# simongroeger/irm_motion_planning

Hardware: AMD Instinct MI355X
Metric: GD iterations/sec (batch of trajectories) (higher is better)
Workload: dtype f32

## Files before the change

### irm_motion_planning_amd/csrc/irm_kernels_impl.hpp

```cpp
#pragma once
#include <hip/hip_runtime.h>
#include <math.h>
#include <stdint.h>
#include <stdio.h>

#include <type_traits>

#include "irm_kernels.hpp"

namespace irm {

typedef float f32x4 __attribute__((ext_vector_type(4)));
typedef float f32x2 __attribute__((ext_vector_type(2)));

__device__ __forceinline__ f32x2 pkfma(f32x2 a, f32x2 b, f32x2 c) { return __builtin_elementwise_fma(a, b, c); }


template <int CTRL>
__device__ __forceinline__ float dppf(float v) {
    static_assert(CTRL == 0xB1 || CTRL == 0x4E || CTRL == 0x141 || CTRL == 0x140, "in-row permutations only");
    return __int_as_float(__builtin_amdgcn_mov_dpp(__float_as_int(v), CTRL, 0xF, 0xF, true));
}
template <int CTRL>
__device__ __forceinline__ int dppi(int v) {
// ... 2626 lines not shown
                } else {
                    G = *reinterpret_cast<const f32x4*>(Gb + ycl * lde + u * 16 + r4y);
                }
                tile(u, G, fresh, *reinterpret_cast<const f32x4*>(Ab + ycl * lde + u * 16 + r4y),
                     vt_frag(u));
            }
        }
        *reinterpret_cast<f32x4*>(Zq + pz * 256 + (r4 >> 2) * 64 + cl * 4) = acc0 + acc1;
    };
    auto bls_f = [&]() {
        const float* zq = Zq + (r4 >> 2) * 64 + cl * 4;
        f32x4 by0, bz;
        if constexpr (kBFix) {
            f32x4 yp[S::NSPLIT], zz[kNZc];
#pragma unroll
            for (int sp = 0; sp < S::NSPLIT; ++sp) yp[sp] = *reinterpret_cast<const f32x4*>(Ypart + (sp * 16 + ycl) * ldy + r4y);
#pragma unroll
            for (int w = 0; w < kNZc; ++w) zz[w] = *reinterpret_cast<const f32x4*>(zq + w * 256);
            __builtin_amdgcn_sched_barrier(0);
            by0 = yp[0];
#pragma unroll
            for (int sp = 1; sp < S::NSPLIT; ++sp) by0 += yp[sp];
            bz = zz[0];
#pragma unroll
            for (int w = 1; w < kNZc; ++w) bz += zz[w];
        } else {
            by0 = *reinterpret_cast<const f32x4*>(Ypart + ycl * ldy + r4y);
            for (int sp = 1; sp < nsplit; ++sp) by0 += *reinterpret_cast<const f32x4*>(Ypart + (sp * 16 + ycl) * ldy + r4y);
            bz = *reinterpret_cast<const f32x4*>(zq);
            for (int w = 1; w < nzp; ++w) bz += *reinterpret_cast<const f32x4*>(zq + w * 256);
        }
        const f32x4 bt = by0 + bz;
        f32x4 acc[S2T];
#pragma unroll
        for (int j = 0; j < S2T; ++j) {
            acc[j] = f32x4{0.f, 0.f, 0.f, 0.f};
            if (wave + j * nwaves < MT2) {
#pragma unroll
                for (int m = 0; m < 4; ++m) acc[j] = __builtin_amdgcn_mfma_f32_16x16x4f32(a2[j * 2][m], bt[m], acc[j], 0, 0, 0);
            }
        }
#pragma unroll
        for (int j = 0; j < S2T; ++j)
            if (wave + j * nwaves < MT2) *reinterpret_cast<f32x4*>(dP + cl * ldx + (wave + j * nwaves) * 16 + r4x) = acc[j];
    };
    constexpr int kDW = MAXT / 64;
    constexpr int kD1 = DENSE ? (S::RP / 16 + kDW - 1) / kDW : 1;
    constexpr int kD2 = DENSE ? (S::MP / 16 + kDW - 1) / kDW : 1;
    constexpr int kDQ = DENSE ? S::NK / 16 : 1;
    constexpr int kDPF = 2;
    float aepd[kD1];
#pragma unroll
    for (int j = 0; j < kD1; ++j) {
        const int tl = wave + j * kDW;
        aepd[j] = 0.f;
        if (DENSE && tl < RP / 16 && (lane >> 4) < 2) aepd[j] = P.Fbot[(size_t)((lane >> 4) ? N - 1 : 0) * RP + tl * 16 + (lane & 15)];
    }
    auto dense_stage1 = [&](bool full) {
        const f32x4 z4 = {0.f, 0.f, 0.f, 0.f};
        constexpr int KQ1c = S::MP / 16;
        const __amdgpu_buffer_rsrc_t r1 = __builtin_amdgcn_make_buffer_rsrc(
            const_cast<float*>(P.F1p), 0, (int)(frag_floats(S::RP, S::MP) * 4), 0x00020000);
        const int vo = lane * 16;
        auto g1ld = [&](int tl, int kq) { return ld_frag(r1, vo, ((tl * KQ1c + kq) * 64) * 16); };
        const float* xl = X + cl * ldx + r4x;
        const float bep = smem[epoff];
        f32x4 acc[kD1];
#pragma unroll
        for (int j = 0; j < kD1; ++j) acc[j] = __builtin_amdgcn_mfma_f32_16x16x4f32(aepd[j], bep, z4, 0, 0, 0);
        auto half = [&](int kb) {
            f32x4 a[kDPF][kD1], b[kDPF];
#pragma unroll
            for (int p = 0; p < kDPF; ++p) {
#pragma unroll
                for (int j = 0; j < kD1; ++j) a[p][j] = g1ld(wave + j * kDW, kb + p);
                b[p] = *reinterpret_cast<const f32x4*>(xl + (kb + p) * 16);
            }
#pragma unroll
            for (int kq = 0; kq < kDQ; ++kq) {
                const int sl = kq % kDPF;
                f32x4 ac[kD1];
#pragma unroll
                for (int j = 0; j < kD1; ++j) ac[j] = a[sl][j];
                const f32x4 bc = b[sl];
                if (kq + kDPF < kDQ) {
#pragma unroll
                    for (int j = 0; j < kD1; ++j) a[sl][j] = g1ld(wave + j * kDW, kb + kq + kDPF);
                    b[sl] = *reinterpret_cast<const f32x4*>(xl + (kb + kq + kDPF) * 16);
                }
#pragma unroll
                for (int m = 0; m < 4; ++m)
#pragma unroll
                    for (int j = 0; j < kD1; ++j) acc[j] = __builtin_amdgcn_mfma_f32_16x16x4f32(ac[j][m], bc[m], acc[j], 0, 0, 0);
                __builtin_amdgcn_sched_barrier(0);
            }
        };
        half(0);
        if (full) half(kDQ);
#pragma unroll
        for (int j = 0; j < kD1; ++j)
            *reinterpret_cast<f32x4*>(Ypart + cl * ldy + (wave + j * kDW) * 16 + r4x) = acc[j];
    };
    auto dense_stage2 = [&]() {
        constexpr int KQ2c = S::RP / 16;
        const __amdgpu_buffer_rsrc_t r2 = __builtin_amdgcn_make_buffer_rsrc(
            const_cast<float*>(P.F2p), 0, (int)(frag_floats(S::MP, S::RP) * 4), 0x00020000);
        const int vo = lane * 16;
        auto g2ld = [&](int tl, int kq) { return ld_frag(r2, vo, ((tl * KQ2c + kq) * 64) * 16); };
        const float* yl = Ypart + cl * ldy + r4x;
        const float* el = Eb + cl * lde + r4x;
        f32x4 acc[kD2], a[kDPF][kD2], by[kDPF], be[kDPF];
#pragma unroll
        for (int j = 0; j < kD2; ++j) acc[j] = f32x4{0.f, 0.f, 0.f, 0.f};
#pragma unroll
        for (int p = 0; p < kDPF; ++p) {
#pragma unroll
            for (int j = 0; j < kD2; ++j) a[p][j] = g2ld(wave + j * kDW, p);
            by[p] = *reinterpret_cast<const f32x4*>(yl + p * 16);
            be[p] = *reinterpret_cast<const f32x4*>(el + p * 16);
        }
#pragma unroll
        for (int kq = 0; kq < kDQ; ++kq) {
            const int sl = kq % kDPF;
            f32x4 ac[kD2];
#pragma unroll
            for (int j = 0; j < kD2; ++j) ac[j] = a[sl][j];
            const f32x4 bt = by[sl] + be[sl];
            if (kq + kDPF < kDQ) {
#pragma unroll
                for (int j = 0; j < kD2; ++j) a[sl][j] = g2ld(wave + j * kDW, kq + kDPF);
                by[sl] = *reinterpret_cast<const f32x4*>(yl + (kq + kDPF) * 16);
                be[sl] = *reinterpret_cast<const f32x4*>(el + (kq + kDPF) * 16);
            }
#pragma unroll
            for (int m = 0; m < 4; ++m)
#pragma unroll
                for (int j = 0; j < kD2; ++j) acc[j] = __builtin_amdgcn_mfma_f32_16x16x4f32(ac[j][m], bt[m], acc[j], 0, 0, 0);
            __builtin_amdgcn_sched_barrier(0);
        }
#pragma unroll
        for (int j = 0; j < kD2; ++j)
            *reinterpret_cast<f32x4*>(dP + cl * ldx + (wave + j * kDW) * 16 + r4x) = acc[j];
    };
    auto direction = [&](int j, float (&dt)[D], float (&dv)[D]) {
        float ut[D], uv[D];
#pragma unroll
        for (int k = 0; k < D; ++k) {
            ut[k] = dP[(t * D + k) * ldx + swz(nn[j], t * D + k)];
            uv[k] = dP[(t * D + k) * ldx + NK + swz(nn[j], t * D + k)];
        }
#pragma unroll
        for (int k = 0; k < D; ++k) {
            float a = ut[0] * P.J[k], c = uv[0] * P.J[k];
#pragma unroll
            for (int l = 1; l < D; ++l) {
                a = fmaf(ut[l], P.J[l * D + k], a);
                c = fmaf(uv[l], P.J[l * D + k], c);
            }
            dt[k] = a;
            dv[k] = c;
        }
    };
    auto grad_alpha = [&](int j, float (&G)[D], int gt) {
        const int r = wl[j] ? nn[j] : 0;
#pragma unroll
        for (int k = 0; k < D; ++k) {
            if constexpr (DENSE) G[k] = Ypart[(gt * D + k) * ldy + swz(r, gt * D + k)];
            else G[k] = Gb[(gt * D + k) * lde + swz(r, gt * D + k)];
        }
    };
    auto ser_row = [&](int j) {
        int r = nn[j] * D;
        if constexpr (D > 3) asm volatile("" : "+v"(r));
        return r;
    };
    auto snapshot = [&](irm_stats& st) {
        if (rec && st.series_len < P.max_series) {
#pragma unroll
            for (int j = 0; j < WPL; ++j) {
                if (vl[j]) {
#pragma unroll
                    for (int k = 0; k < D; ++k)
                        P.series[((b * P.max_series) + st.series_len) * N * D + ser_row(j) + k] = q[j][k];
                }
            }
            st.series_len++;
        }
    };

    float* SS = smem + LX.ss;
    float* HP = smem + LX.hp;
    constexpr int kSlots = (MAXT / 64) / WPTL;
    auto ss_write = [&](int tt, const float (&a)[WPL][D], const float (&qq)[WPL][D], const float (&vv)[WPL][D]) {
        const int th = tt * NWL + li;
#pragma unroll
        for (int k = 0; k < D; ++k) {
            SS[k * MAXT + th] = a[0][k];
            SS[(D + k) * MAXT + th] = qq[0][k];
            SS[(2 * D + k) * MAXT + th] = vv[0][k];
        }
    };
    auto ss_read = [&](int tt) {
        const int th = tt * NWL + li;
#pragma unroll
        for (int k = 0; k < D; ++k) {
            al[0][k] = SS[k * MAXT + th];
            q[0][k] = SS[(D + k) * MAXT + th];
            v[0][k] = SS[(2 * D + k) * MAXT + th];
        }
    };
    bool adopt = false;
    bool qpend = false;
    auto ts_write = [&]() {
        if (n0 == 0 && lane == 0) {
            TS[t * kTsW + 0] = lr;
            TS[t * kTsW + 2] = phase == LP_STEP ? 1.f : 0.f;
            if constexpr (QUE) TS[t * kTsW + 3] = __int_as_float((int)b);
        }
    };
    int n_rounds = 0, n_hm = 0;

    irm_stats st{};
    st.series_len = rec ? 1 : 0;
    if constexpr (BLS && D <= 3) {
        asm volatile("" : "+v"(st.inner_iterations), "+v"(st.outer_iterations), "+v"(st.grad_evals), "+v"(st.cost_evals),
                     "+v"(st.bls_trials), "+v"(st.series_len), "+v"(n_rounds), "+v"(n_hm));
    }
    auto write_out = [&]() {
#pragma unroll
        for (int j = 0; j < WPL; ++j) {
            if (vl[j]) {
#pragma unroll
                for (int k = 0; k < D; ++k) {
                    if (P.traj_out) P.traj_out[(b * N + nn[j]) * D + k] = q[j][k];
                    if (P.alpha_out) P.alpha_out[(b * N + nn[j]) * D + k] = al[j][k];
                }
            }
        }
        if (P.stats && li == 0) P.stats[b] = st;
    };

    float loss;
    bool done = !tvalid;
    {
        WP<D> w[WPL];
        evaluate(q, v, false, ljl, w);
        __syncthreads();
        const Fin f = finalize(lsg, t);
        loss = f.nl;
        if constexpr (!BLS) st.cost_evals = 1;
        bool to_end = P.max_inner <= 0;
        if constexpr (BLS) to_end = to_end || P.max_outer <= 0;
        bool bfar = false;
        if constexpr (GD1) {
            if (to_end) done = true;
        } else if (to_end) {
            phase = LP_RESYNC;
            st.final_loss = loss;
        } else {
            needs_dir = true;
        }
        if (!done && !to_end) {
            bfar = grad_inputs(w, q, v, f.idx, lsg, ljl, t);
            xdense = bfar;
        }
        if constexpr (BLS) {
            if (tvalid) ts_write();
        }
        if constexpr (kHelp) {
            if (tvalid) {
                if constexpr (!kSSLazy) ss_write(t, al, q, v);
                if (n0 == 0 && lane == 0) {
                    HP[t * kHpW + 0] = lr;
                    HP[t * kHpW + 1] = ljl;
                    HP[t * kHpW + 2] = lsg;
                    HP[t * kHpW + 3] = loss;
                    HP[t * kHpW + 4] = __int_as_float(0);
                    HP[t * kHpW + 5] = __int_as_float(0);
                }
            }
        }
        if constexpr (GD1) {
            if (lane == 0 && (!done || bfar)) atomicOr(&fw[0], (done ? 0u : 1u << wave) | (bfar ? 1u << 31 : 0u));
        } else {
            if (lane == 0 && tvalid)
                atomicOr(&fw[0], (1u << wave) | (needs_dir ? 1u << 28 : 0u) | (phase == LP_RESYNC ? 1u << 29 : 0u) |
                                     (phase == LP_STEP ? 1u << 30 : 0u) |
                                     ((BLS ? xdense && phase == LP_STEP : bfar) ? 1u << 31 : 0u));
        }
    }
    __syncthreads();

    IRM_STAMP(14);
    constexpr bool kReloadOps = D > 3 && MAXT > 256;
#ifndef IRM_X_RESYNC_U
    constexpr int kResyncU = (D <= 3 && WPL == 1) ? 8 : 2;
#else
    constexpr int kResyncU = (D <= 3 && WPL == 1) ? IRM_X_RESYNC_U : 2;
#endif
    if (wave >= 4) __builtin_amdgcn_s_setprio(1);
#ifdef IRM_X_PRIO_RESTORE
    bool hm_prev = false;
#endif
    for (int par = 0;; par ^= 1) {
        f32x4 pre1[KQU1], pre1w[KQU1];
        f32x4 zpre[kZPre ? kKQZ : 1];
        zpre_load(zpre);
        float pre1e = 0.f;
        unsigned flw = 0u;
        if constexpr (kS1Ord) {
            const unsigned flv = fw[par];
            __builtin_amdgcn_sched_barrier(0);
            if (has1) {
                stage1_load(pre1, pre1w, pre1e);
                asm volatile("v_readfirstlane_b32 %0, %1 ; flag word, stage-1 waves" : "=s"(flw) : "v"(flv));
            } else {
                asm volatile("v_readfirstlane_b32 %0, %1 ; flag word, other waves" : "=s"(flw) : "v"(flv));
            }
        }
        if constexpr (kPre1 && !kS1Ord) stage1_load(pre1, pre1w, pre1e);
        const unsigned fl = kS1Ord ? flw : fw[par];
        if constexpr (GD1) {
            if ((fl & 0x7FFFFFFFu) == 0u) break;
        } else {
            if ((fl & 0xFFFFu) == 0u) break;
        }
        const bool dense = (fl >> 31) != 0u;
        const bool dirr = GD1 || ((fl >> 28) & 1u);
        const bool rsy = !GD1 && ((fl >> 29) & 1u);
        if constexpr (!kS1Ord) {
            if (tid == 0) fw[par ^ 1] = 0u;
        }
        if constexpr (QUE) {
            if (qpend) {
                const int nx = __builtin_amdgcn_readfirstlane(__float_as_int(red[(t * WPTL) * 8 + 6]));
                qpend = false;
                if (nx < P.B) {
                    b = (size_t)nx;
                    phase = LP_LOAD;
                }
            }
        }
        bool hm = false, helper = false;
        int ts = 0, hs = 0;
        float h_lr0 = 0.f, h_lr = 0.f, h_ljl = 0.f, h_lsg = 0.f, h_loss = 0.f, h_gn = 1.f, h_an = 0.f;
        int h_trial = 0, h_inner = 0;
        if constexpr (kHelp) {
            n_rounds++;
            if (adopt) {
                ss_read(t);
                xdense = HP[t * kHpW + 6 + (wave - t * WPTL)] != 0.f;
                adopt = false;
            }
            if (!rec && !P.lean_nohelp && ((fl >> 30) & 1u) && kSlots > 1) {
                unsigned live = 0u;
#pragma unroll
                for (int s2 = 0; s2 < kSlots; ++s2)
                    if ((fl >> (s2 * WPTL)) & ((1u << WPTL) - 1u)) live |= 1u << s2;
                if (__builtin_popcount(live) == 1) {
                    hm = true;
                    n_hm++;
                    ts = __builtin_ctz(live);
                    hs = ts ^ 1;
                    if ((hs + 1) * D > kCols) hs = ts - 1;
                    helper = t == hs;
                }
            }
            ycl = (hm && cl / D == hs) ? ts * D + cl % D : cl;
            r4y = r4 ^ (ycl & 4);
            if (hm) {
                if (t == ts) __builtin_amdgcn_s_setprio(3);
                else __builtin_amdgcn_s_setprio(0);
            }
#ifdef IRM_X_PRIO_RESTORE
            else if (hm_prev) {
                if (wave >= 4) __builtin_amdgcn_s_setprio(1);
                else __builtin_amdgcn_s_setprio(0);
            }
            hm_prev = hm;
#endif
            if constexpr (kSSLazy) {
                if (hm && t == ts) ss_write(t, al, q, v);
            }
            if (helper) {
                if constexpr (!kSSLazy) ss_read(ts);
                const size_t bs = QUE ? (size_t)__float_as_int(TS[ts * kTsW + 3]) : (size_t)(tb0 + ts);
#pragma unroll
                for (int k = 0; k < D; ++k) tg[0][k] = (nn[0] == N - 1) ? P.goal[bs * D + k] : P.start[bs * D + k];
                vl[0] = wl[0];
                obs = obsL + (P.obs_stride ? ts * obs_pitch(P.O) : 0);
                if constexpr (OREG) {
                    if (P.obs_stride && obs_reg) {
#pragma unroll
                        for (int i = 0; i < 6; ++i) oreg[i] = reinterpret_cast<const f32x4*>(obs)[i];
                    }
                }
                h_lr0 = HP[ts * kHpW + 0];
                h_lr = h_lr0 * P.bls_bm;
                h_ljl = HP[ts * kHpW + 1];
                h_lsg = HP[ts * kHpW + 2];
                h_loss = HP[ts * kHpW + 3];
                h_trial = dirr ? 0 : __float_as_int(HP[ts * kHpW + 4]);
                h_inner = __float_as_int(HP[ts * kHpW + 5]);
            }
        }
        IRM_STAMP(0);
        if constexpr (!BLS) {
            if (dirr) {
                IRM_COUNT(13, dense);
                if constexpr (DENSE) {
                    dense_stage1(dense);
                } else {
                    stage1(dense, pre1, pre1w, pre1e);
                    stage1z(zpre);
                    if constexpr (kS1Ord) {
                        if (tid == 0) fw[par ^ 1] = 0u;
                    }
                }
                IRM_STAMP(1);
                __syncthreads();
                IRM_STAMP(2);
                if constexpr (DENSE) dense_stage2();
                else stage2f(std::true_type{}, std::true_type{});
                IRM_STAMP(3);
                __syncthreads();
                IRM_STAMP(4);
                if constexpr (kGLate) glate_tiles();
            }
        } else if ((fl >> 30) & 1u) {
            if (dirr) {
                IRM_COUNT(13, dense);
                stage1(dense, pre1, pre1w, pre1e);
                IRM_STAMP(1);
                __syncthreads();
                IRM_STAMP(2);
            }
            if (dirr) bls_gz(std::true_type{}, hm, hs);
            else bls_gz(std::false_type{}, hm, hs);
            if (dirr) {
                if (needs_dir && n0 == 0) {
                    float s1 = 0.f;
                    if (tvalid && li < RP) {
                        float sa = 0.f;
                        const int lr = lnd(li);
#pragma unroll
                        for (int a = 0; a < D; ++a) {
                            float y = Ypart[(t * D + a) * ldy + swz(lr, t * D + a)];
                            for (int sp = 1; sp < nsplit; ++sp) y += Ypart[(sp * 16 + t * D + a) * ldy + swz(lr, t * D + a)];
                            sa += y;
                        }
                        s1 = sa * sa;
                    }
                    s1 = wred_sum(s1);
                    if (lane == 0) wp[t * 2 + 1] = s1;
                }
            }
            IRM_STAMP(3);
            __syncthreads();
            IRM_STAMP(4);
            if constexpr (kSSLazy) {
                if (helper) ss_read(ts);
            }
            bls_f();
            __syncthreads();
        }
        if constexpr (BLS) {
            if (needs_dir) {
                gnorm = TS[t * kTsW + 1];
                anorm = wp[t * 2 + 1] / gnorm;
                st.grad_evals++;
                st.cost_evals++;
                trial = 0;
                needs_dir = false;
            }
        }
        float cj = cfac, stepj = lr, lrj = lr, gnj = gnorm;
        if constexpr (BLS) {
            if (helper) {
                h_gn = TS[ts * kTsW + 1];
                h_an = wp[ts * 2 + 1] / h_gn;
                lrj = h_lr;
                gnj = h_gn;
            }
            cj = unfused(1.f - unfused(P.lreg * lrj));
            stepj = div_rcp(lrj, gnj, rcp_refined(gnj));
        }
        if (rsy) {
            const bool rs = phase == LP_RESYNC || (QUE && phase == LP_LOAD);
            if constexpr (QUE) {
                if (phase == LP_LOAD) {
                    vl[0] = nn[0] < N;
#pragma unroll
                    for (int k = 0; k < D; ++k) tg[0][k] = (nn[0] == N - 1) ? P.goal[b * D + k] : P.start[b * D + k];
                    if (P.alpha0) {
#pragma unroll
                        for (int k = 0; k < D; ++k) al[0][k] = vl[0] ? P.alpha0[(b * N + nn[0]) * D + k] : 0.f;
                    } else {
                        const float un = vl[0] ? P.uvec[nn[0]] : 0.f, wn = vl[0] ? P.wvec[nn[0]] : 0.f;
#pragma unroll
                        for (int k = 0; k < D; ++k) {
                            float sj = 0.f, gj = 0.f;
#pragma unroll
                            for (int e2 = 0; e2 < D; ++e2) {
                                sj += P.start[b * D + e2] * P.Jinv[e2 * D + k];
                                gj += P.goal[b * D + e2] * P.Jinv[e2 * D + k];
                            }
                            al[0][k] = vl[0] ? un * sj + wn * gj : 0.f;
                        }
                    }
                    if constexpr (BLS) {
                        if (vl[0]) {
#pragma unroll
                            for (int k = 0; k < D; ++k) Ab[(t * D + k) * lde + swz(nn[0], t * D + k)] = al[0][k];
                        }
                    }
                    obs = obsL + (P.obs_stride ? t * obs_pitch(P.O) : 0);
                    if (P.obs_stride) {
                        const int pitch = obs_pitch(P.O);
                        for (int r = li; r < pitch; r += NWL) {
                            const int o = 2 * (r >> 2) + (r & 1), coord = (r >> 1) & 1;
                            obsL[t * pitch + r] = o < P.O ? P.obstacles[b * P.obs_stride + 2 * o + coord] : 1.0e20f;
                        }
                    }
                    lsg = P.lsg0;
                    ljl = P.ljl0;
                    lr = BLS ? P.bls_lr0 : P.gd_lr[0];
                    cfac = P.gd_c[0];
                    gnorm = 1.f;
                    anorm = 0.f;
                    outer = inner = trial = 0;
                    needs_dir = xdense = adopt = false;
                    n_rounds = n_hm = 0;
                    st = irm_stats{};
                }
            }
            if (rs) {
#pragma unroll
                for (int j = 0; j < WPL; ++j) {
                    if (vl[j]) {
#pragma unroll
                        for (int k = 0; k < D; ++k) {
                            X[(t * D + k) * ldx + lnd(nn[j])] = al[j][k];
                            if constexpr (!BLS) Eb[(t * D + k) * lde + swz(nn[j], t * D + k)] = 0.f;
                        }
                    }
                }
            }
            __syncthreads();
            if constexpr (QUE && OREG) {
                if (phase == LP_LOAD && P.obs_stride && obs_reg) {
#pragma unroll
                    for (int i = 0; i < 6; ++i) oreg[i] = reinterpret_cast<const f32x4*>(obs)[i];
                }
            }
            if (rs) {
#pragma unroll
                for (int j = 0; j < WPL; ++j) {
                    if (vl[j]) {
                        if constexpr (D <= 3) eval_exact<D, kResyncU, true>(P, X + (t * D) * ldx, nn[j], q[j], v[j], nullptr, nullptr, 1, ldx, Jl);
                        else eval_exact_loop<D, 4>(P, X + (t * D) * ldx, ldx, nn[j], N, Jl, q[j], v[j]);
                        if (rec && st.series_len > 0) {
#pragma unroll
                            for (int k = 0; k < D; ++k)
                                P.series[((b * P.max_series) + st.series_len - 1) * N * D + ser_row(j) + k] = q[j][k];
                        }
                    }
                }
            }
            if constexpr (kReloadOps) {
                asm volatile("" ::: "memory");
                load_ops();
            }
            __syncthreads();
        }
        float q2[WPL][D], v2[WPL][D];
        WP<D> w[WPL];
#ifdef IRM_X_GPRE
        constexpr bool kGPre = !BLS;
#else
        constexpr bool kGPre = GD1 && D <= 3 && !kGLate;
#endif
        float Gp[kGPre ? WPL : 1][D];
        constexpr bool kAjPre = BLS;
        float Ajp[kAjPre ? WPL : 1][D];
        const bool stepping = GD1 ? !done : (phase == LP_STEP || helper);
        const bool ev = GD1 ? !done : (phase != LP_DONE || helper);
        if (ev) {
#pragma unroll
            for (int j = 0; j < WPL; ++j) {
                if (stepping) {
                    float dt[D], dv[D];
                    {
                        direction(j, dt, dv);
                        if constexpr (kGPre) grad_alpha(j, Gp[j], t);
                        if constexpr (kAjPre) {
#pragma unroll
                            for (int k = 0; k < D; ++k) Ajp[j][k] = Ajb[(t * D + k) * lde + swz(wl[j] ? lnd(nn[j]) : 0, t * D + k)];
                        }
#pragma unroll
                        for (int k = 0; k < D; ++k) {
                            const float tq = -(stepj * dt[k]), tv = -(stepj * dv[k]);
                            q2[j][k] = fmaf(cj, q[j][k], tq);
                            v2[j][k] = fmaf(cj, v[j][k], tv);
                            if constexpr (GD1) asm volatile("" ::"v"(tq), "v"(tv), "v"(q2[j][k]), "v"(v2[j][k]));
                        }
                    }
                } else {
// ... 697 lines not shown
```

Measured before the change: 342.0 million.

## Add specialized all-live fast loop for C3 kernel when every slot is active

Adds a dedicated inner gradient-descent loop, used when all trajectory slots are live under the C3 configuration. It drops the generic per-phase branching (direction resync, phase flags, reload checks) and runs a lean sequence of stage1, stage2, evaluate, finalize and accept/reject. On rejection or when a slot finishes, it falls back to the general loop at the correct parity. The aim is to cut control overhead and branching per iteration, at the cost of duplicated logic that must stay consistent with the general loop's bookkeeping.

```diff
diff --git a/irm_motion_planning_amd/csrc/irm_kernels_impl.hpp b/irm_motion_planning_amd/csrc/irm_kernels_impl.hpp
--- a/irm_motion_planning_amd/csrc/irm_kernels_impl.hpp
+++ b/irm_motion_planning_amd/csrc/irm_kernels_impl.hpp
@@ -2952,7 +2952,130 @@
 #ifdef IRM_X_PRIO_RESTORE
     bool hm_prev = false;
 #endif
-    for (int par = 0;; par ^= 1) {
+    int par0 = 0;
+    if constexpr (kTopC3) {
+        constexpr int kW1 = (S::RP / 16) * S::NSPLIT;
+        static_assert(kW1 + kZS == MAXT / 64 && kZFix && !kZPre && kGLate && kGFin && kLatF && kAllLive && kLeanKeep<D>,
+                      "the all-live loop is written for C3's kernel");
+        if (ntb == kSlots) {
+            constexpr unsigned kAllW = (1u << (MAXT / 64)) - 1u;
+            const unsigned wbit = 1u << wave;
+            const LeanW cw = lean_weights(P, ljl);
+            const f32x4 zpre[1] = {f32x4{0.f, 0.f, 0.f, 0.f}};
+            float llr = P.llr;
+            asm volatile("" : "+s"(llr));
+            int rnd = 0;
+            bool rej = false;
+            int par = 0;
+            for (;; par ^= 1) {
+                f32x4 pre1[KQU1], pre1w[KQU1];
+                float pre1e = 0.f;
+                unsigned fl = 0u;
+                const unsigned flv = fw[par];
+                __builtin_amdgcn_sched_barrier(0);
+                if (has1) {
+                    stage1_load(pre1, pre1w, pre1e);
+                    asm volatile("v_readfirstlane_b32 %0, %1 ; flag word, stage-1 waves (all-live)" : "=s"(fl) : "v"(flv));
+                    if ((fl & kAllW) != kAllW) break;
+                    IRM_STAMP(0);
+                    IRM_COUNT(13, (fl >> 31) != 0u);
+                    stage1((fl >> 31) != 0u, pre1, pre1w, pre1e);
+                    if (wave == 0) fw[par ^ 1] = 0u;
+                } else {
+                    asm volatile("v_readfirstlane_b32 %0, %1 ; flag word, z waves (all-live)" : "=s"(fl) : "v"(flv));
+                    if ((fl & kAllW) != kAllW) break;
+                    stage1z(zpre);
+                }
+                IRM_STAMP(1);
+                __syncthreads();
+                IRM_STAMP(2);
+                stage2f(std::true_type{}, std::true_type{});
+                IRM_STAMP(3);
+                __syncthreads();
+                IRM_STAMP(4);
+                glate_tiles();
+                float q2[WPL][D], v2[WPL][D];
+                WP<D> w[WPL];
+                {
+                    float dt[D], dv[D];
+                    direction(0, dt, dv);
+#pragma unroll
+                    for (int k = 0; k < D; ++k) {
+                        const float tq = -(lr * dt[k]), tv = -(lr * dv[k]);
+                        q2[0][k] = fmaf(cfac, q[0][k], tq);
+                        v2[0][k] = fmaf(cfac, v[0][k], tv);
+                        asm volatile("" ::"v"(tq), "v"(tv), "v"(q2[0][k]), "v"(v2[0][k]));
+                    }
+                }
+                IRM_STAMP(5);
+#pragma unroll
+                for (int k = 0; k < D; ++k) {
+                    q[0][k] = q2[0][k];
+                    v[0][k] = v2[0][k];
+                }
+                evaluate(q2, v2, false, ljl, w);
+                IRM_STAMP(7);
+                __syncthreads();
+                IRM_STAMP(8);
+                float Gf[D];
+                grad_alpha(0, Gf, t);
+                const Fin f = finalize(lsg, t);
+                IRM_STAMP(9);
+                if (loss - f.nl < llr) {
+                    rej = true;
+                    par ^= 1;
+                    IRM_STAMP(11);
+                    __syncthreads();
+                    IRM_STAMP(12);
+                    break;
+                } else {
+                    loss = f.nl;
+                    float eo[D];
+#pragma unroll
+                    for (int k = 0; k < D; ++k) al[0][k] = alpha_step_gd2(al[0][k], cfac, lr, Gf[k], nilr, eo[k]);
+#pragma unroll
+                    for (int k = 0; k < D; ++k) Eb[(t * D + k) * lde + swz(nn[0], t * D + k)] = eo[k];
+                    if (rnd + 1 < P.max_inner) {
+                        const int n = nn[0];
+                        float a[D], bb[D], ep[D];
+                        grad_waypoint_lean<D>(P, w[0], q2[0], v2[0], n == f.idx, epf[0] * lsg, cw, tg[0], a, bb);
+                        unsigned zb = 0u;
+#pragma unroll
+                        for (int k = 0; k < D; ++k) {
+                            float ma = 0.f, mb = 0.f;
+#pragma unroll
+                            for (int d = 0; d < D; ++d) {
+                                ma = fmaf(a[d], P.J[k * D + d], ma);
+                                mb = fmaf(bb[d], P.J[k * D + d], mb);
+                            }
+                            X[(t * D + k) * ldx + swz(n, t * D + k)] = ma;
+                            X[(t * D + k) * ldx + NK + swz(n, t * D + k)] = mb;
+                            zb |= __float_as_uint(w[0].zvm[k]);
+                            ep[k] = mb;
+                        }
+                        const bool bfar = (__ballot(zb != 0u) & ~endm[0]) != 0ull;
+                        if (epf[0] != 0.f) {
+                            float* e = EPt + (n == 0 ? 0 : kEpS);
+#pragma unroll
+                            for (int k = 0; k < D; ++k) e[k] = ep[k];
+                        }
+                        if (lane == 0) atomicOr(&fw[par ^ 1], wbit | (bfar ? 1u << 31 : 0u));
+                    }
+                }
+                ++rnd;
+                IRM_STAMP(11);
+                __syncthreads();
+                IRM_STAMP(12);
+            }
+            par0 = par;
+            st.grad_evals += rnd + (rej ? 1 : 0);
+            st.cost_evals += rnd + (rej ? 1 : 0);
+            st.inner_iterations += rnd;
+            inner += rnd;
+            if (rej || inner >= P.max_inner) done = true;
+        }
+    }
+    for (int par = par0;; par ^= 1) {
         f32x4 pre1[KQU1], pre1w[KQU1];
         f32x4 zpre[kZPre ? kKQZ : 1];
         zpre_load(zpre);
```

Result: faster. 354.7 million, median of 6 (+3.7%).
